# cristicbz/rust-doom

Measured on NVIDIA H100. Metric: frames/sec at 1920x1080 (palette-index bit-exact), higher is better.
Workload: dtype u8

## Files before the change

rust-doom_b200/csrc/b2d_kernels.cu:

```cuda
#include "b2d_kernels.cuh"

namespace b2d {

namespace {

constexpr unsigned kFull = 0xFFFFFFFFu;

constexpr int kMaskWords = 128;
constexpr int kStackDepth = 128;

constexpr uint32_t kVisBit = 1u << 25, kSolidBit = 1u << 24;
__device__ __forceinline__ uint32_t pack_range(int lo, int hi, uint32_t bits) {
    return (uint32_t)lo | ((uint32_t)hi << 12) | bits;
}
__device__ __forceinline__ int range_lo(uint32_t r) { return (int)(r & 0xFFFu); }
__device__ __forceinline__ int range_hi(uint32_t r) { return (int)((r >> 12) & 0xFFFu); }

__device__ __forceinline__ uint32_t word_bits(int w, int lo, int hi) {
    int a = max(lo, w * 32), b = min(hi, w * 32 + 31);
    if (a > b) return 0u;
    uint32_t m = 0xFFFFFFFFu >> (31 - (b - w * 32));
    return m & (0xFFFFFFFFu << (a - w * 32));
}

// ... 166 lines not shown
        if (--budget < 0) { status |= kStatusNoTermination; break; }
        uint32_t child = stack[--sp];
        __syncwarp();
        if (child & kLeaf) {
            uint32_t id = child & 0x7FFFFFFFu;
            if (id >= (uint32_t)sc.nss) continue;
            const int4 ssv = ssec_s[id];
            SSectorRec ss;
            ss.first_seg = ssv.x; ss.num_segs = ssv.y; ss.sector = ssv.z; ss.sprites = ssv.w;
            if (ss.sector < 0) continue;
            {
                const int sfirst = ss.sprites & 0xFFFFFF;
                int scnt = (ss.sprites >> 24) & 0xFF;
                if (sfirst + scnt > sc.nsprites) scnt = sc.nsprites > sfirst ? sc.nsprites - sfirst : 0;
                int nvis = 0;
                for (int k0 = 0; k0 < scnt; k0 += 32) {
                    const int k = k0 + lane, pi = sfirst + k;
                    const uint32_t r = k < scnt ? sprr[pi] : 0u;
                    const bool vis = (r & kVisBit) && lane_range_open(mask, range_lo(r), range_hi(r));
                    int rank = 0, total = 0;
                    const int32_t myz = vis ? sprz[pi] : 0;
                    for (int j0 = 0; j0 < scnt; j0 += 32) {
                        const int j = j0 + lane, pj = sfirst + j;
                        const uint32_t rj = j < scnt ? sprr[pj] : 0u;
                        const bool vj = (rj & kVisBit) && lane_range_open(mask, range_lo(rj), range_hi(rj));
                        const int32_t zj = vj ? sprz[pj] : 0;
                        unsigned mj = __ballot_sync(kFull, vj);
                        total += __popc(mj);
                        while (mj) {
                            const int b = __ffs(mj) - 1;
                            mj &= mj - 1;
                            const int32_t zb = __shfl_sync(kFull, zj, b);
                            const int jb = j0 + b;
                            if (vis && (zb < myz || (zb == myz && jb < k))) rank++;
                        }
                    }
                    const int pos = count + rank;
                    if (vis && pos < sc.nsegs + sc.nsprites) list[pos] = (uint16_t)(sc.nsegs + pi);
                    nvis = total;
                }
                count = min(count + nvis, sc.nsegs + sc.nsprites);
                __syncwarp();
            }
            for (int k0 = 0; k0 < ss.num_segs; k0 += 32) {
                int k = k0 + lane;
                int si = ss.first_seg + k;
                uint32_t r = k < ss.num_segs ? segr[si] : 0u;
                bool vis = (r & kVisBit) && lane_range_open(mask, range_lo(r), range_hi(r));
                unsigned m = __ballot_sync(kFull, vis);
                int pos = count + __popc(m & ((1u << lane) - 1u));
                if (vis && pos < sc.nsegs + sc.nsprites) list[pos] = (uint16_t)si;
                count = min(count + __popc(m), sc.nsegs + sc.nsprites);
                unsigned sm = __ballot_sync(kFull, vis && (r & kSolidBit));
                __syncwarp();
                while (sm) {
                    int j = __ffs(sm) - 1;
                    sm &= sm - 1;
                    uint32_t rj = __shfl_sync(kFull, r, j);
                    mark_solid(mask, lane, range_lo(rj), range_hi(rj), passes);
                }
                __syncwarp();
            }
            if (!range_open(mask, lane, 0, vw.W - 1, passes)) break;
        } else {
            if (child >= (uint32_t)sc.nnodes) continue;
            const int4 nl = node_s[2 * child], nc = node_s[2 * child + 1];
            int side = node_side(fc.pose, nl.x, nl.y, nl.z, nl.w);
            uint32_t near_c = (uint32_t)(side ? nc.y : nc.x), far_c = (uint32_t)(side ? nc.x : nc.y);
            uint32_t rn = boxr[2 * child + side], rf = boxr[2 * child + (side ^ 1)];
            bool far_vis = (rf & kVisBit) && range_open(mask, lane, range_lo(rf), range_hi(rf), passes);
            bool near_vis = (rn & kVisBit) && range_open(mask, lane, range_lo(rn), range_hi(rn), passes);
            int need = (far_vis ? 1 : 0) + (near_vis ? 1 : 0);
            if (sp + need > kStackDepth) { status = kStatusStackOverflow; break; }
            if (lane == 0) {
                int p = sp;
                if (far_vis) stack[p++] = far_c;
                if (near_vis) stack[p++] = near_c;
            }
            sp += need;
            __syncwarp();
        }
    }
    __syncwarp();
    if (warp == 0 && lane == 0) {
        if (count > stride) { count = stride; status |= kStatusWorklistFull; }
        s_count = count; s_status = status;
    }
    __syncthreads();
    count = s_count; status = s_status;

    for (int k = tid; k < count; k += nthr) {
        int si = list[k];
        SegFrame sf;
        if (si >= sc.nsegs) {
            const int pi = si - sc.nsegs;
            const SpriteRec &P = state_table<kStates>(sc.sprites, tb, st.off_sprites)[pi];
            SpriteFrame sp;
            sprite_setup(fc, vw, P.x, P.y, (int32_t)state_table<kStates>(sc.tex, tb, 0u)[P.tex].w, sp);
            sprite_entry(pi, sp, sf);
            work[(size_t)frame * stride + k] = sf;
            continue;
        }
        const SegRec &S = state_table<kStates>(sc.segs, tb, st.off_segs)[si];
        seg_frame_setup(vw, tx[S.v1], tz[S.v1], tx[S.v2], tz[S.v2], sf, false);
        sf.seg = si;
        work[(size_t)frame * stride + k] = sf;
    }
    if (tid == 0) {
        if (status) atomicOr(sc.status_flag, status);
        fc.count = count;
        fc.status = status;
#pragma unroll
        for (int i = 0; i < 6; i++) fc.pad[i] = 0;
        if (kStates) fc.pad[0] = (int32_t)slot;
        frames[frame] = fc;
    }
    __syncthreads();
    }
}

__device__ __forceinline__ uint32_t lds_u32(uint32_t a) {
    uint32_t v;
    asm("ld.shared.u32 %0, [%1];" : "=r"(v) : "r"(a));
    return v;
}

struct RasterCtx {
    const DeviceScene *sc;
    uint32_t pal_s;
    uint2 *rowz;
    PlaneDir dir;
    uint8_t *fb;
    uint32_t *rgba;
    int W, H, x, lane;
    uint32_t skycol;
};

template <bool kRgba>
__device__ __forceinline__ void put_px(const RasterCtx &c, uint8_t *p8, uint32_t *p32, bool on, uint32_t v) {
    if (on) {
        if (kRgba) {
            *p8 = (uint8_t)v;
            *p32 = lds_u32(c.pal_s + 4u * v);
        } else {
            __stcs(p8, (uint8_t)v);
        }
    }
}

__host__ __device__ __forceinline__ bool tex_interleaved(const TexRec &T) { return b2d::tex_interleaved(T.h, T.texel_off); }

constexpr int kBatch = 8;

template <bool kRgba, int kW>
__device__ __forceinline__ void store_batch(const RasterCtx &c, uint8_t *p8, uint32_t *p32, const uint32_t (&v)[kBatch],
                                            int y, int ya, int yb, bool full) {
    const int Wc = kW ? kW : c.W;
    if (full) {
#pragma unroll
        for (int k = 0; k < kBatch; k++) put_px<kRgba>(c, p8 + (size_t)k * Wc, kRgba ? p32 + (size_t)k * Wc : nullptr, true, v[k]);
    } else {
        const uint32_t m = row_mask(y, ya, yb, kBatch);
#pragma unroll
        for (int k = 0; k < kBatch; k++)
            put_px<kRgba>(c, p8 + (size_t)k * Wc, kRgba ? p32 + (size_t)k * Wc : nullptr, (m >> k) & 1u, v[k]);
    }
}

template <bool kRgba, int kW>
__device__ __forceinline__ void fill_void_warp(const RasterCtx &c, int ya, int yb) {
    bool act = ya < yb;
    int y0 = __reduce_min_sync(kFull, act ? ya : 0x7FFFFFFF);
    int y1 = __reduce_max_sync(kFull, act ? yb : 0);
    if (y0 >= y1) return;
    const int Wc = kW ? kW : c.W;
    uint8_t *p8 = c.fb + (size_t)y0 * Wc;
    uint32_t *p32 = kRgba ? c.rgba + (size_t)y0 * Wc : nullptr;
#pragma unroll 1
    for (int y = y0; y < y1; y++, p8 += Wc, p32 += Wc) put_px<kRgba>(c, p8, p32, y >= ya && y < yb, 0u);
}

template <bool kRgba, int kW>
__device__ __forceinline__ void draw_sky_warp(const RasterCtx &c, int ya, int yb) {
    const DeviceScene &sc = *c.sc;
    if (sc.sky_tex < 0) { fill_void_warp<kRgba, kW>(c, ya, yb); return; }
    const TexRec T = sc.tex[sc.sky_tex];
    const bool inter = tex_interleaved(T);
    const uint8_t *px = sc.lit_texels + T.texel_off + (inter ? 4u * c.skycol : c.skycol);
    const uint32_t w4 = 4u * T.w;
    bool act = ya < yb;
    int y0 = __reduce_min_sync(kFull, act ? ya : 0x7FFFFFFF);
    int y1 = __reduce_max_sync(kFull, act ? yb : 0);
    if (y0 >= y1) return;
    const int Wc = kW ? kW : c.W;
    uint8_t *p8 = c.fb + (size_t)y0 * Wc;
    uint32_t *p32 = kRgba ? c.rgba + (size_t)y0 * Wc : nullptr;
#pragma unroll 2
    for (int y = y0; y < y1; y++, p8 += Wc, p32 += Wc) {
        const uint32_t r = sc.skyrow[y];
        put_px<kRgba>(c, p8, p32, y >= ya && y < yb, __ldg(px + (inter ? (r >> 2) * w4 + (r & 3u) : r * T.w)));
    }
}

template <bool kRgba, int kW>
__device__ __forceinline__ void draw_plane_warp(const RasterCtx &c, const FrameConst &fc, const View &vw,
                                                int ya, int yb, int32_t h, int32_t flat, int lightb,
                                                bool visible) {
    const DeviceScene &sc = *c.sc;
    if (!__any_sync(kFull, ya < yb)) return;
    if (!visible) { fill_void_warp<kRgba, kW>(c, ya, yb); return; }
    if (flat == kFlatSky) { draw_sky_warp<kRgba, kW>(c, ya, yb); return; }
    if (flat < 0 || flat >= sc.nflats) { fill_void_warp<kRgba, kW>(c, ya, yb); return; }
    const uint64_t px_hi = reinterpret_cast<uint64_t>(sc.lit_flats) & 0xFFFFFFFF00000000ull;
    const uint32_t habs = plane_habs(h, fc.pose.z);
    bool act = ya < yb;
    int y0 = __reduce_min_sync(kFull, act ? ya : 0x7FFFFFFF);
    int y1 = __reduce_max_sync(kFull, act ? yb : 0);
    const int full_lo = __reduce_max_sync(kFull, act ? ya : 0x7FFFFFFF);
    const int full_hi = __reduce_min_sync(kFull, act ? yb : 0);
    const int Wc = kW ? kW : c.W;
    uint8_t *p8 = c.fb + (size_t)y0 * Wc;
    uint32_t *p32 = kRgba ? c.rgba + (size_t)y0 * Wc : nullptr;
    const uint32_t bu = (uint32_t)fc.pose.x << 10, bv = (uint32_t)fc.pose.y << 10;
    const uint32_t ax = (uint32_t)c.dir.ax, ay = (uint32_t)c.dir.ay;
    for (int yc = y0; yc < y1; yc += 32) {
        int yy = yc + c.lane;
        if (yy < y1) {
            const PlaneRow pr = plane_row(habs, sc.yslope[yy]);
            c.rowz[c.lane] = make_uint2(pr.z8q, (sc.lit_flat_stride >> 6) * (uint32_t)light_row(lightb, pr.z8) + 64u * (uint32_t)flat);
        }
        __syncwarp();
        const int rows = min(32, y1 - yc);
        int j = 0;
        for (; j + kBatch <= rows; j += kBatch, p8 += (size_t)kBatch * Wc, p32 += (size_t)kBatch * Wc) {
            uint32_t v[kBatch];
#pragma unroll
            for (int k = 0; k < kBatch; k++) {
                const uint2 rz = c.rowz[j + k];
                v[k] = __ldg(reinterpret_cast<const uint8_t *>(px_hi | flat_offset(rz.y, bu + rz.x * ax, bv + rz.x * ay)));
            }
            const int y = yc + j;
            store_batch<kRgba, kW>(c, p8, p32, v, y, ya, yb, y >= full_lo && y + kBatch <= full_hi);
        }
        for (; j < rows; j++, p8 += Wc, p32 += Wc) {
            const uint2 rz = c.rowz[j];
            const int y = yc + j;
            put_px<kRgba>(c, p8, p32, y >= ya && y < yb,
                          __ldg(reinterpret_cast<const uint8_t *>(px_hi | flat_offset(rz.y, bu + rz.x * ax, bv + rz.x * ay))));
        }
        __syncwarp();
    }
}

template <bool kRgba, int kW, int R>
__device__ __forceinline__ void wall_fast_loop(const RasterCtx &c, const uint8_t *plq, uint32_t w4, uint32_t nq, uint32_t q,
                                               uint32_t acc, uint32_t ts29, int y0, int y1, int ya, int yb,
                                               int full_lo, int full_hi) {
    const int Wc = kW ? kW : c.W;
    uint8_t *p8 = c.fb + (size_t)y0 * Wc;
    uint32_t *p32 = kRgba ? c.rgba + (size_t)y0 * Wc : nullptr;
    asm("" : "+l"(plq));
#pragma unroll 1
    for (int y = y0; y < y1; y += R, p8 += (size_t)R * Wc, p32 += (size_t)R * Wc) {
        const uint32_t q1 = q + 1u == nq ? 0u : q + 1u;
        const uint32_t w0 = __ldg(reinterpret_cast<const uint32_t *>(plq + (size_t)q * w4));
        const uint32_t w1 = __ldg(reinterpret_cast<const uint32_t *>(plq + (size_t)q1 * w4));
        if (y >= full_lo && y + R <= full_hi) {
#pragma unroll
            for (int k = 0; k < R; k++) {
                uint32_t v = pick_byte(w0, w1, wall_sel(acc, ts29, (uint32_t)k));
                if (kRgba) v &= 0xFFu;
                put_px<kRgba>(c, p8 + (size_t)k * Wc, kRgba ? p32 + (size_t)k * Wc : nullptr, true, v);
            }
        } else {
            const uint32_t m = row_mask(y, ya, yb, R);
#pragma unroll
            for (int k = 0; k < R; k++) {
                uint32_t v = pick_byte(w0, w1, wall_sel(acc, ts29, (uint32_t)k));
                if (kRgba) v &= 0xFFu;
                put_px<kRgba>(c, p8 + (size_t)k * Wc, kRgba ? p32 + (size_t)k * Wc : nullptr, (m >> k) & 1u, v);
            }
        }
        wall_advance(acc, q, ts29, (uint32_t)R, nq);
    }
}

template <bool kRgba, int kW>
__device__ __forceinline__ void draw_wall_warp(const RasterCtx &c, const FrameConst &fc, int ya, int yb,
                                               int32_t tex, int32_t tA, int32_t hA, int32_t ucol,
                                               int32_t iscale, int row) {
    const DeviceScene &sc = *c.sc;
    if (!__any_sync(kFull, ya < yb)) return;
    if (tex < 0 || tex >= sc.ntex) { fill_void_warp<kRgba, kW>(c, ya, yb); return; }
    const TexRec T = sc.tex[tex];
    bool act = ya < yb;
    const uint32_t col = (uint32_t)floormod32(ucol, (int32_t)T.w);
    const uint8_t *pl = sc.lit_texels + (size_t)row * sc.lit_texel_stride + T.texel_off;
    const uint32_t tstep = (uint32_t)(iscale >> 4);
    int y0 = __reduce_min_sync(kFull, act ? ya : 0x7FFFFFFF);
    int y1 = __reduce_max_sync(kFull, act ? yb : 0);
    const int full_lo = __reduce_max_sync(kFull, act ? ya : 0x7FFFFFFF);
    const int full_hi = __reduce_min_sync(kFull, act ? yb : 0);
    uint32_t t = (uint32_t)wall_tbase(tA, hA, fc.pose.z, c.H, iscale) + (uint32_t)y0 * tstep;
    const int Wc = kW ? kW : c.W;
    uint8_t *p8 = c.fb + (size_t)y0 * Wc;
    uint32_t *p32 = kRgba ? c.rgba + (size_t)y0 * Wc : nullptr;
    if (tex_interleaved(T) && T.h >= 8u) {
        const uint32_t ts = act ? tstep : 0u;
        const bool f16 = __all_sync(kFull, ts <= kWallFast16);
        if (f16 || __all_sync(kFull, ts <= kWallFast8)) {
            const uint32_t tt = act ? t : 0u;
            const uint32_t r0 = wall_row((int32_t)tt, T.h, T.hmagic, T.hbias);
            const uint8_t *plq = pl + 4u * col;
            if (f16) wall_fast_loop<kRgba, kW, 16>(c, plq, 4u * T.w, T.h >> 2, r0 >> 2, wall_acc29(tt, r0), ts << 13, y0, y1, ya, yb, full_lo, full_hi);
            else wall_fast_loop<kRgba, kW, 8>(c, plq, 4u * T.w, T.h >> 2, r0 >> 2, wall_acc29(tt, r0), ts << 13, y0, y1, ya, yb, full_lo, full_hi);
            return;
        }
    }
    if (tex_interleaved(T)) {
        const uint32_t colb = 4u * col, w4 = 4u * T.w;
        for (int y = y0; y < y1; y += kBatch, p8 += (size_t)kBatch * Wc, p32 += (size_t)kBatch * Wc, t += (uint32_t)kBatch * tstep) {
            const uint32_t r0 = wall_row((int32_t)t, T.h, T.hmagic, T.hbias);
            const uint32_t acc = wall_acc(t, r0);
            const uint32_t b7 = (acc + 7u * tstep) >> 16;
            uint32_t v[kBatch];
            if (__all_sync(kFull, b7 < 8u)) {
                const uint32_t q0 = r0 >> 2, q1 = next_quad(q0, T.h);
                const uint32_t w0 = __ldg(reinterpret_cast<const uint32_t *>(pl + (q0 * w4 + colb)));
                const uint32_t w1 = __ldg(reinterpret_cast<const uint32_t *>(pl + (q1 * w4 + colb)));
#pragma unroll
                for (int k = 0; k < kBatch; k++) {
                    v[k] = pick_byte(w0, w1, (acc + (uint32_t)k * tstep) >> 16);
                    if (kRgba) v[k] &= 0xFFu;
                }
            } else {
                const uint32_t t4 = t + 4u * tstep;
                const uint32_t r4 = wall_row((int32_t)t4, T.h, T.hmagic, T.hbias);
                const uint32_t acc4 = wall_acc(t4, r4);
                if (__all_sync(kFull, ((acc + 3u * tstep) >> 16) < 8u && ((acc4 + 3u * tstep) >> 16) < 8u)) {
                    const uint32_t q0 = r0 >> 2, q4 = r4 >> 2;
                    const uint32_t a0 = __ldg(reinterpret_cast<const uint32_t *>(pl + (q0 * w4 + colb)));
                    const uint32_t a1 = __ldg(reinterpret_cast<const uint32_t *>(pl + (next_quad(q0, T.h) * w4 + colb)));
                    const uint32_t b0 = __ldg(reinterpret_cast<const uint32_t *>(pl + (q4 * w4 + colb)));
                    const uint32_t b1 = __ldg(reinterpret_cast<const uint32_t *>(pl + (next_quad(q4, T.h) * w4 + colb)));
#pragma unroll
                    for (int k = 0; k < 4; k++) {
                        v[k] = pick_byte(a0, a1, (acc + (uint32_t)k * tstep) >> 16);
                        v[k + 4] = pick_byte(b0, b1, (acc4 + (uint32_t)k * tstep) >> 16);
                        if (kRgba) { v[k] &= 0xFFu; v[k + 4] &= 0xFFu; }
                    }
                } else {
#pragma unroll
                    for (int k = 0; k < kBatch; k++) {
                        const uint32_t rk = wall_row((int32_t)(t + (uint32_t)k * tstep), T.h, T.hmagic, T.hbias);
                        v[k] = __ldg(pl + ((rk >> 2) * w4 + colb + (rk & 3u)));
                    }
                }
            }
            store_batch<kRgba, kW>(c, p8, p32, v, y, ya, yb, y >= full_lo && y + kBatch <= full_hi);
        }
    } else {
        const uint8_t *px = pl + col;
#pragma unroll 1
        for (int y = y0; y < y1; y++, p8 += Wc, p32 += Wc, t += tstep)
            put_px<kRgba>(c, p8, p32, y >= ya && y < yb, __ldg(px + wall_row((int32_t)t, T.h, T.hmagic, T.hbias) * T.w));
    }
}

__device__ __forceinline__ uint32_t *masked_entry(const DeviceScene &sc, const uint32_t *chunks, int e) {
    return sc.masked_list + ((size_t)chunks[e / kMaskedChunk] * kMaskedChunk + (size_t)(e % kMaskedChunk)) * 33u;
}
__device__ __forceinline__ uint32_t *masked_push(const DeviceScene &sc, uint32_t *chunks, int &mcount, int lane) {
    bool ok = mcount < sc.masked_cap;
    if (ok && mcount % kMaskedChunk == 0) {
        uint32_t id = 0;
        if (lane == 0) id = atomicAdd(sc.masked_counter, 1u);
        id = __shfl_sync(kFull, id, 0);
        ok = id < sc.masked_chunks;
        if (ok && lane == 0) chunks[mcount / kMaskedChunk] = id;
        __syncwarp();
    }
    if (!ok) {
        if (lane == 0) atomicOr(sc.status_flag, kStatusMaskedFull);
        return nullptr;
    }
    return masked_entry(sc, chunks, mcount++);
}

template <bool kRgba, int kW, bool kStates>
__device__ __noinline__ void masked_pass(const DeviceScene &sc, const View &vw, int32_t pose_z, uint8_t *fb,
                                         uint32_t *rgba, uint32_t pal_s, int x, int lane,
                                         const SegFrame *wl, const uint32_t *chunks, int count) {
    RasterCtx c;
    c.sc = &sc; c.pal_s = pal_s; c.fb = fb; c.rgba = rgba;
    c.W = vw.W; c.H = vw.H; c.x = x; c.lane = lane;
    const int Wc = kW ? kW : c.W;
    for (int e = count - 1; e >= 0; e--) {
        const uint32_t *ml = masked_entry(sc, chunks, e);
        const uint32_t k = ml[0];
        const uint32_t packed = ml[1 + c.lane];
        int ya = (int)(packed & 0xFFFFu), yb = (int)(packed >> 16);
        const SegFrame sf = wl[k];
        int32_t tex, tA, hA, ucol = 0, iscale = 1, row = 0;
        if (is_sprite_entry(sf)) {
            SpriteFrame sp;
            const SpriteRec P = sc.sprites[entry_sprite(sf, sp)];
            if (P.tex < 0 || P.tex >= sc.ntex) continue;
            const int32_t sw = (int32_t)sc.tex[P.tex].w, sh = (int32_t)sc.tex[P.tex].h;
            const int64_t scale = sprite_scale(vw, sp.cz);
            int32_t z8;
            scale_depth(vw, scale, iscale, z8);
            row = light_row_sprite(P.light, z8);
            tex = P.tex; tA = 0; hA = P.low + sh;
            if (ya < yb) {
                clip_rows(P.low + sh, P.low, (int32_t)scale, pose_z, c.H, ya, yb);
                ucol = sprite_column(sp, vw, c.x, sw);
            }
        } else {
            const SegRec S = sc.segs[sf.seg];
            if (S.mid < 0 || S.mid >= sc.nmids) continue;
            const MidRec M = sc.mids[S.mid];
            tex = M.tex; tA = M.t_high; hA = M.high;
            ColumnEval ce = {0u, 1, 1, 0};
            if (ya < yb && column_eval(sf, vw, c.x, ce)) {
                clip_rows(M.high, M.low, ce.scale, pose_z, c.H, ya, yb);
                ucol = wall_column(S.uoff, S.len_q12, ce.s24);
                iscale = ce.iscale;
                row = light_row(S.light, ce.z8);
            } else {
                ya = yb = 0;
            }
        }
        if (tex < 0 || tex >= sc.ntex) continue;
        const TexRec T = sc.tex[tex];
        const bool act = ya < yb;
        int y0 = __reduce_min_sync(kFull, act ? ya : 0x7FFFFFFF);
        int y1 = __reduce_max_sync(kFull, act ? yb : 0);
        if (y0 >= y1) continue;
        const uint32_t col = (uint32_t)floormod32(ucol, (int32_t)T.w);
        const bool inter = tex_interleaved(T);
        const bool has_mask = T.mask_off != 0xFFFFFFFFu;
        const uint8_t *pl = sc.lit_texels + (size_t)row * sc.lit_texel_stride + T.texel_off;
        const uint8_t *pm = sc.lit_texels + (size_t)32 * sc.lit_texel_stride + T.texel_off;
        const uint32_t tstep = (uint32_t)(iscale >> 4);
        uint32_t t = (uint32_t)wall_tbase(tA, hA, pose_z, c.H, iscale) + (uint32_t)y0 * tstep;
        uint8_t *p8 = c.fb + (size_t)y0 * Wc;
        uint32_t *p32 = kRgba ? c.rgba + (size_t)y0 * Wc : nullptr;
        const uint32_t len = act ? (uint32_t)(yb - ya) : 0u;
        if (inter) {
            const uint32_t colb = 4u * col, w4 = 4u * T.w;
#pragma unroll 1
            for (int y = y0; y < y1; y += kBatch, p8 += (size_t)kBatch * Wc, p32 += (size_t)kBatch * Wc, t += (uint32_t)kBatch * tstep) {
                const uint32_t r0 = wall_row((int32_t)t, T.h, T.hmagic, T.hbias);
                const uint32_t acc = wall_acc(t, r0);
                const uint32_t d = (uint32_t)(y - ya);
                uint32_t v[kBatch], o[kBatch];
                if (__all_sync(kFull, ((acc + 7u * tstep) >> 16) < 8u)) {
                    const uint32_t o0 = (r0 >> 2) * w4 + colb, o1 = next_quad(r0 >> 2, T.h) * w4 + colb;
                    const uint32_t w0 = __ldg(reinterpret_cast<const uint32_t *>(pl + o0));
                    const uint32_t w1 = __ldg(reinterpret_cast<const uint32_t *>(pl + o1));
                    uint32_t m0 = 0x01010101u, m1 = 0x01010101u;
                    if (has_mask) {
                        m0 = __ldg(reinterpret_cast<const uint32_t *>(pm + o0));
                        m1 = __ldg(reinterpret_cast<const uint32_t *>(pm + o1));
                    }
#pragma unroll
                    for (int k = 0; k < kBatch; k++) {
                        const uint32_t bk = (acc + (uint32_t)k * tstep) >> 16;
                        v[k] = pick_byte(w0, w1, bk) & 0xFFu;
                        o[k] = pick_byte(m0, m1, bk) & 0xFFu;
                    }
                } else {
#pragma unroll
                    for (int k = 0; k < kBatch; k++) {
                        const uint32_t rk = wall_row((int32_t)(t + (uint32_t)k * tstep), T.h, T.hmagic, T.hbias);
                        const uint32_t off = (rk >> 2) * w4 + colb + (rk & 3u);
                        v[k] = __ldg(pl + off);
                        o[k] = has_mask ? (uint32_t)__ldg(pm + off) : 1u;
                    }
                }
#pragma unroll
                for (int k = 0; k < kBatch; k++)
                    put_px<kRgba>(c, p8 + (size_t)k * Wc, kRgba ? p32 + (size_t)k * Wc : nullptr, d + (uint32_t)k < len && o[k] != 0u, v[k]);
            }
        } else {
#pragma unroll 1
            for (int y = y0; y < y1; y++, p8 += Wc, p32 += Wc, t += tstep) {
                const uint32_t off = wall_row((int32_t)t, T.h, T.hmagic, T.hbias) * T.w + col;
                const bool on = (uint32_t)(y - ya) < len && (!has_mask || __ldg(pm + off) != 0);
                put_px<kRgba>(c, p8, p32, on, __ldg(pl + off));
            }
        }
    }
}

constexpr int kRasterWarps = 4;

template <bool kRgba, int kW, bool kMasked, bool kStates>
__global__ void __launch_bounds__(32 * kRasterWarps, 16 / kRasterWarps)
b2d_raster_kernel(const __grid_constant__ DeviceScene sc, const __grid_constant__ View vw, const FrameConst *__restrict__ frames,
                  const SegFrame *__restrict__ work, int stride, int n, int strips,
                  uint8_t *__restrict__ index_fb, uint32_t *__restrict__ rgba_fb, const __grid_constant__ StateTables st) {
    __shared__ uint32_t s_pal[kRgba ? 256 : 1];
    __shared__ uint2 s_rowz[kRasterWarps][32];
    __shared__ uint32_t s_chunks[kRasterWarps][kMasked ? kMaskedCapMax / kMaskedChunk : 1];
    if (kRgba) {
        for (int i = threadIdx.x; i < 256; i += blockDim.x) s_pal[i] = sc.palette[i];
        __syncthreads();
    }

    const int lane = threadIdx.x & 31;
    const long long gw = (long long)blockIdx.x * (blockDim.x >> 5) + (threadIdx.x >> 5);
    if (gw >= (long long)n * strips) return;
    const int frame = (int)(gw / strips), strip = (int)(gw % strips);
    const int W = kW ? kW : vw.W, H = vw.H;
    const int x0 = strip * 32, x = x0 + lane;
    const bool inside = x < W;

    const FrameConst fc = frames[frame];
    const DeviceScene *scp = &sc;
    if constexpr (kStates) {
        __shared__ DeviceScene s_sc[kRasterWarps];
        DeviceScene *d = &s_sc[threadIdx.x >> 5];
        const uint32_t *src = reinterpret_cast<const uint32_t *>(&sc);
        uint32_t *dst = reinterpret_cast<uint32_t *>(d);
        for (int i = lane; i < (int)(sizeof(DeviceScene) / 4); i += 32) dst[i] = src[i];
        __syncwarp();
        if (lane == 0) {
            const uint8_t *tb = st.base + (size_t)(uint32_t)fc.pad[0] * st.slot_bytes;
            d->tex = reinterpret_cast<const TexRec *>(tb);
            d->sectors = reinterpret_cast<const SectorRec *>(tb + st.off_sectors);
            d->segs = reinterpret_cast<const SegRec *>(tb + st.off_segs);
            d->sprites = reinterpret_cast<const SpriteRec *>(tb + st.off_sprites);
            d->mids = reinterpret_cast<const MidRec *>(tb + st.off_mids);
        }
        __syncwarp();
        scp = d;
    }
    const DeviceScene &ts = *scp;
    RasterCtx c;
    c.sc = &ts;
    c.pal_s = (uint32_t)__cvta_generic_to_shared(s_pal);
    c.rowz = s_rowz[threadIdx.x >> 5];
    c.dir = plane_dir(fc, vw, inside ? x : 0, sc.invF);
    c.fb = index_fb + (size_t)frame * W * H + (inside ? x : 0);
    c.rgba = kRgba ? rgba_fb + (size_t)frame * W * H + (inside ? x : 0) : nullptr;
    c.W = W; c.H = H; c.x = x; c.lane = lane;
    c.skycol = 0;
    if (sc.sky_tex >= 0 && inside) c.skycol = umulhi32(sky_u32(x, vw, fc.pose.angle), ts.tex[sc.sky_tex].w);

    int ct = 0, cb = inside ? H : 0;
    uint32_t *chunks = s_chunks[threadIdx.x >> 5];
    asm("" : "+l"(chunks));
    const bool defer = kMasked && sc.masked_list != nullptr;
    int mcount = 0;
    const SegFrame *wl = work + (size_t)frame * stride;
    const int count = fc.count;
    bool done = false;

    for (int k0 = 0; k0 < count && !done; k0 += 32) {
        int k = k0 + lane;
        bool overlap = false;
        if (k < count) {
            int xlo = wl[k].xlo, xhi = wl[k].xhi;
            overlap = xhi >= x0 && xlo <= x0 + 31;
        }
        unsigned m = __ballot_sync(kFull, overlap);
        while (m) {
            int j = __ffs(m) - 1;
            m &= m - 1;
            if (!__any_sync(kFull, ct < cb)) { done = true; break; }
            const SegFrame sf = wl[k0 + j];
            bool in = inside && ct < cb && x >= sf.xlo && x <= sf.xhi;
            if (!__any_sync(kFull, in)) continue;
            if (is_sprite_entry(sf)) {
                if (defer) {
                    uint32_t *ml = masked_push(sc, chunks, mcount, lane);
                    if (ml) {
                        if (lane == 0) ml[0] = (uint32_t)(k0 + j);
                        ml[1 + lane] = in ? ((uint32_t)ct | ((uint32_t)cb << 16)) : 0u;
                    }
                }
                continue;
            }
            ColumnEval ce = {0u, 1, 1, 0};
            bool ok = in && column_eval(sf, vw, x, ce);
            if (!__any_sync(kFull, ok)) continue;

            const SegRec S = ts.segs[sf.seg];
            const SectorRec SF = ts.sectors[S.front];
            const int32_t fcl = SF.ceil, ffl = SF.floor;
            const bool two = S.flags & kSegTwoSided;
            const bool ceil_vis = plane_visible(true, fcl, SF.ceil_flat == kFlatSky, fc.pose.z);
            const bool floor_vis = plane_visible(false, ffl, SF.floor_flat == kFlatSky, fc.pose.z);

            WallRows wr = {ct, ct, ct, ct};
            int yend = ct, row = 0;
            int32_t ucol = 0;
            if (ok) {
                row = light_row(S.light, ce.z8);
                ucol = wall_column(S.uoff, S.len_q12, ce.s24);
                wr = wall_rows(fcl, ffl, two, S.otop, S.obot, ce.scale, fc.pose.z, H, ct, cb);
                yend = cb;
            }
#pragma unroll 1
            for (int pz = 0; pz < 2; pz++) {
                const bool top = pz == 0;
                draw_plane_warp<kRgba, kW>(c, fc, vw, ok ? (top ? ct : wr.y4) : 0, ok ? (top ? wr.y1 : yend) : 0,
                                                    top ? fcl : ffl, top ? SF.ceil_flat : SF.floor_flat, SF.light,
                                                    top ? ceil_vis : floor_vis);
            }
#pragma unroll 1
            for (int pw = 0; pw < 2; pw++) {
                const bool upper = pw == 0;
                if (!wall_piece(upper, two, fcl, ffl, S.otop, S.obot)) continue;
                draw_wall_warp<kRgba, kW>(c, fc, ok ? (upper ? wr.y1 : wr.y3) : 0, ok ? (upper ? wr.y2 : wr.y4) : 0,
                                                   upper ? S.texA : S.texB, upper ? S.tA : S.tB, upper ? S.hA : S.hB,
                                                   ucol, ce.iscale, row);
            }
            if (ok) wall_window(two, wr, H, ct, cb);
            if (defer && two && S.mid >= 0) {
                const bool keep = ok && wr.y2 < wr.y3;
                if (__any_sync(kFull, keep)) {
                    uint32_t *ml = masked_push(sc, chunks, mcount, lane);
                    if (ml) {
                        if (lane == 0) ml[0] = (uint32_t)(k0 + j);
                        ml[1 + lane] = keep ? ((uint32_t)wr.y2 | ((uint32_t)wr.y3 << 16)) : 0u;
                    }
                }
            }
        }
    }
    fill_void_warp<kRgba, kW>(c, inside ? ct : 0, inside ? cb : 0);
    if (kMasked && mcount > 0) {
        __syncwarp();
        masked_pass<kRgba, kW, kStates>(ts, vw, fc.pose.z, c.fb, c.rgba, c.pal_s, x, lane, wl, chunks, mcount);
    }
}

__global__ void __launch_bounds__(256)
b2d_palette_kernel(const uint32_t *__restrict__ palette, const uint8_t *__restrict__ index,
                   uint32_t *__restrict__ rgba, size_t n_pixels) {
    __shared__ uint32_t s_pal[256];
    s_pal[threadIdx.x] = palette[threadIdx.x];
    __syncthreads();
    const bool aligned = ((reinterpret_cast<uintptr_t>(index) | reinterpret_cast<uintptr_t>(rgba)) & 15) == 0;
    const size_t nvec = aligned ? n_pixels / 16 : 0;
    const size_t stride = (size_t)gridDim.x * blockDim.x;
    for (size_t i = (size_t)blockIdx.x * blockDim.x + threadIdx.x; i < nvec; i += stride) {
        uint4 in = __ldcs(reinterpret_cast<const uint4 *>(index) + i);
        uint32_t wds[4] = {in.x, in.y, in.z, in.w};
        uint4 *out = reinterpret_cast<uint4 *>(rgba) + 4 * i;
#pragma unroll
        for (int q = 0; q < 4; q++) {
            uint4 o;
            o.x = s_pal[wds[q] & 0xFF];
            o.y = s_pal[(wds[q] >> 8) & 0xFF];
            o.z = s_pal[(wds[q] >> 16) & 0xFF];
            o.w = s_pal[wds[q] >> 24];
            __stcs(out + q, o);
        }
    }
    for (size_t p = nvec * 16 + (size_t)blockIdx.x * blockDim.x + threadIdx.x; p < n_pixels; p += stride)
        rgba[p] = s_pal[index[p]];
}

}

size_t walk_smem_per_warp(const DeviceScene &sc) { return walk_layout(sc.nverts, sc.nsegs, sc.nnodes, sc.nss, sc.nsprites).total; }

static int device_sms() {
    int dev = 0, sms = 0;
    cudaGetDevice(&dev);
    cudaDeviceGetAttribute(&sms, cudaDevAttrMultiProcessorCount, dev);
    return sms > 0 ? sms : 1;
}

cudaError_t launch_walk(const DeviceScene &sc, const View &vw, const Pose *d_poses, int n,
                        FrameConst *d_frames, SegFrame *d_work, int stride, cudaStream_t stream, bool background,
                        const StateTables *states) {
    if (n <= 0) return cudaSuccess;
    const size_t smem = walk_smem_per_warp(sc);
    if (smem > 227 * 1024) return cudaErrorInvalidValue;
    if (smem > 48 * 1024) {
        cudaError_t e = states ? cudaFuncSetAttribute(b2d_walk_kernel<true>, cudaFuncAttributeMaxDynamicSharedMemorySize, (int)smem)
                               : cudaFuncSetAttribute(b2d_walk_kernel<false>, cudaFuncAttributeMaxDynamicSharedMemorySize, (int)smem);
        if (e != cudaSuccess) return e;
    }
    const int sms = device_sms();
    const int blocks = (background && n > sms) ? sms : n, warps = 4;
    const StateTables none{};
    if (states) b2d_walk_kernel<true><<<blocks, warps * 32, smem, stream>>>(sc, vw, d_poses, n, d_frames, d_work, stride, *states);
    else b2d_walk_kernel<false><<<blocks, warps * 32, smem, stream>>>(sc, vw, d_poses, n, d_frames, d_work, stride, none);
    return cudaGetLastError();
}

cudaError_t launch_raster(const DeviceScene &sc, const View &vw, const FrameConst *d_frames,
                          const SegFrame *d_work, int stride, int n, uint8_t *d_index_fb,
                          uint32_t *d_rgba, cudaStream_t stream, const StateTables *states) {
    if (n <= 0) return cudaSuccess;
    const int strips = (vw.W + 31) / 32;
    const int nblocks = (int)(((long long)n * strips + kRasterWarps - 1) / kRasterWarps);
    const bool masked = (sc.nmids > 0 || sc.nsprites > 0) && sc.masked_list;
    const StateTables none{};
#define B2D_RASTER_GO2(RGBA, KW, KS) do { \
    if (masked) b2d_raster_kernel<RGBA, KW, true, KS><<<nblocks, 32 * kRasterWarps, 0, stream>>>(sc, vw, d_frames, d_work, stride, n, strips, d_index_fb, d_rgba, KS ? *states : none); \
    else b2d_raster_kernel<RGBA, KW, false, KS><<<nblocks, 32 * kRasterWarps, 0, stream>>>(sc, vw, d_frames, d_work, stride, n, strips, d_index_fb, d_rgba, KS ? *states : none); \
    } while (0)
#define B2D_RASTER_GO(RGBA, KW) do { if (states) B2D_RASTER_GO2(RGBA, KW, true); else B2D_RASTER_GO2(RGBA, KW, false); } while (0)
    if (d_rgba) { if (vw.W == 1920) B2D_RASTER_GO(true, 1920); else B2D_RASTER_GO(true, 0); }
    else if (vw.W == 1920) B2D_RASTER_GO(false, 1920);
    else if (vw.W == 3840) B2D_RASTER_GO(false, 3840);
    else B2D_RASTER_GO(false, 0);
#undef B2D_RASTER_GO
#undef B2D_RASTER_GO2
    return cudaGetLastError();
}

namespace {
__global__ void __launch_bounds__(256)
b2d_prelight_kernel(const uint8_t *__restrict__ colormap, const uint8_t *__restrict__ src, uint8_t *__restrict__ dst,
                    size_t n, size_t stride) {
    __shared__ uint8_t cm[32 * 256];
    for (int i = threadIdx.x; i < 32 * 256; i += blockDim.x) cm[i] = colormap[i];
    __syncthreads();
    for (size_t i = (size_t)blockIdx.x * blockDim.x + threadIdx.x; i < n; i += (size_t)gridDim.x * blockDim.x) {
        const uint32_t t = src[i];
#pragma unroll 4
        for (int r = 0; r < 32; r++) dst[(size_t)r * stride + i] = cm[r * 256 + t];
    }
}
}

namespace {
__global__ void __launch_bounds__(256)
b2d_prelight_tex_kernel(const uint8_t *__restrict__ colormap, const uint8_t *__restrict__ texels,
                        const TexRec *__restrict__ tex, int ntex, uint8_t *__restrict__ dst, size_t stride) {
    __shared__ uint8_t cm[32 * 256];
    for (int i = threadIdx.x; i < 32 * 256; i += blockDim.x) cm[i] = colormap[i];
    __syncthreads();
    for (int ti = blockIdx.x; ti < ntex; ti += gridDim.x) {
        const TexRec T = tex[ti];
        const bool inter = tex_interleaved(T);
        const uint32_t n = T.w * T.h;
        for (uint32_t i = threadIdx.x; i < n; i += blockDim.x) {
            const uint32_t row = i / T.w, col = i - row * T.w;
            const uint32_t o = lit_index(inter, T.w, row, col);
            const uint32_t t = texels[T.texel_off + i];
            for (int r = 0; r < 32; r++) dst[(size_t)r * stride + T.texel_off + o] = cm[r * 256 + t];
            if (T.mask_off != 0xFFFFFFFFu) dst[(size_t)32 * stride + T.texel_off + o] = texels[T.mask_off + i];
        }
    }
}
}

cudaError_t launch_prelight_textures(const uint8_t *d_colormap, const uint8_t *d_texels, const TexRec *d_tex, int ntex,
                                     uint8_t *d_dst, size_t stride, cudaStream_t stream) {
    if (ntex <= 0) return cudaSuccess;
    const int cap = device_sms() * 8;
    b2d_prelight_tex_kernel<<<ntex < cap ? ntex : cap, 256, 0, stream>>>(d_colormap, d_texels, d_tex, ntex, d_dst, stride);
    return cudaGetLastError();
// ... 59 lines not shown
```

rust-doom_b200/csrc/b2d_math.cuh:

```cuda
#pragma once
#include <stdint.h>

#if defined(__CUDACC__)
#define B2D_HD __host__ __device__ __forceinline__
#else
#define B2D_HD inline
#endif

namespace b2d {

struct Pose { int32_t x, y, z; uint32_t angle; };
struct View { int32_t W, H, F, FY2; };

struct FrameConst {
    Pose pose;
    int32_t cosq, sinq;
    int32_t px8, py8;
    int32_t count;
    int32_t status;
    int32_t pad[6];
};
static_assert(sizeof(FrameConst) == 64, "FrameConst");

constexpr int32_t kStatusStackOverflow = 1;
// ... 166 lines not shown
    sf.sh = (int16_t)sh;
    sf.e = (int16_t)(5 - sh + shm);
    sf.Dmax = M >> 8;
    sf.flags = 0;
    if (want_noskip) {
        ColumnEval ce;
        bool ok = column_eval(sf, vw, (int)lo, ce) && column_eval(sf, vw, (int)hi, ce);
        sf.flags = ok ? kSegFrameNoSkip : 0;
    }
    sf.pad = 0;
    return true;
}

B2D_HD bool seg_closes(bool two, int32_t otop, int32_t obot) { return !two || otop <= obot; }
B2D_HD bool seg_solid(bool closes, const SegFrame &sf) { return closes && (sf.flags & kSegFrameNoSkip); }

B2D_HD int light_row(int b, int32_t z8) {
    uint32_t Z = (uint32_t)z8 + 720u;
    int32_t num = (int32_t)(64u * (uint32_t)(255 - b) * Z) - 5875200;
    if (num <= 0) return 0;
    uint32_t r = (uint32_t)num / (255u * Z);
    return r > 31u ? 31 : (int)r;
}

B2D_HD int yrow(int32_t h, int32_t scale, int32_t pose_z, int32_t H) {
    int64_t hrel8 = ((int64_t)h << 8) - (int64_t)(pose_z >> 8);
    int64_t Y = ((int64_t)H << 25) - hrel8 * scale;
    int64_t r = (Y + ((int64_t)1 << 25) - 1) >> 26;
    return (int)clampv<int64_t>(r, 0, H);
}

B2D_HD bool plane_visible(bool ceiling, int32_t h, bool sky, int32_t pose_z) {
    const int64_t h16 = (int64_t)h << 16;
    return (ceiling ? h16 > pose_z : h16 < pose_z) || sky;
}
struct WallRows { int y1, y2, y3, y4; };
B2D_HD WallRows wall_rows(int32_t ceil, int32_t floor, bool two, int32_t otop, int32_t obot, int32_t scale, int32_t pose_z,
                          int32_t H, int ct, int cb) {
    WallRows r;
    const int yfc = yrow(ceil, scale, pose_z, H), yff = yrow(floor, scale, pose_z, H);
    r.y1 = clampv(yfc, ct, cb);
    if (!two) {
        r.y2 = clampv(yff, r.y1, cb);
        r.y3 = r.y2; r.y4 = r.y2;
    } else {
        r.y2 = clampv(yrow(otop, scale, pose_z, H), r.y1, cb);
        r.y3 = clampv(yrow(obot, scale, pose_z, H), r.y2, cb);
        r.y4 = clampv(yff, r.y3, cb);
    }
    return r;
}
B2D_HD bool wall_piece(bool upper, bool two, int32_t ceil, int32_t floor, int32_t otop, int32_t obot) {
    return upper ? (!two || otop < ceil) : (two && obot > floor);
}
B2D_HD void wall_window(bool two, const WallRows &r, int32_t H, int &ct, int &cb) {
    if (!two || r.y2 >= r.y3) { ct = H; cb = 0; }
    else { ct = r.y2; cb = r.y3; }
}
B2D_HD int32_t wall_column(int32_t uoff, int32_t len_q12, uint32_t s24) {
    return uoff + (int32_t)(((uint64_t)s24 * (uint32_t)len_q12) >> 36);
}
B2D_HD void clip_rows(int32_t high, int32_t low, int32_t scale, int32_t pose_z, int32_t H, int &ya, int &yb) {
    const int a = yrow(high, scale, pose_z, H), b = yrow(low, scale, pose_z, H);
    if (a > ya) ya = a;
    if (b < yb) yb = b;
}

B2D_HD uint32_t yslope_entry(int y, const View &vw) {
    int32_t r2 = 2 * y + 1 - vw.H;
    if (r2 < 0) r2 = -r2;
    if (r2 == 0) r2 = 1;
    return (uint32_t)(((uint64_t)vw.FY2 << 16) / (uint32_t)r2);
}

B2D_HD uint32_t plane_habs(int32_t h, int32_t pose_z) {
    int64_t hrel = clampv<int64_t>(((int64_t)h << 16) - pose_z, -((int64_t)1 << 27), (int64_t)1 << 27);
    return (uint32_t)(hrel < 0 ? -hrel : hrel);
}
B2D_HD int32_t wall_hrel(int32_t h, int32_t pose_z) {
    return (int32_t)clampv<int64_t>(((int64_t)h << 16) - pose_z, -((int64_t)1 << 27), (int64_t)1 << 27);
}

struct PlaneDir { int32_t ax, ay; };
B2D_HD PlaneDir plane_dir(const FrameConst &f, const View &vw, int x, uint32_t invF) {
    const int64_t c2 = 2 * (int64_t)x + 1 - vw.W;
    const int64_t nx = ((int64_t)f.cosq * vw.F + (int64_t)f.sinq * c2) >> 4;
    const int64_t ny = ((int64_t)f.sinq * vw.F - (int64_t)f.cosq * c2) >> 4;
    PlaneDir d;
    d.ax = (int32_t)((nx * (int64_t)invF) >> 40);
    d.ay = (int32_t)((ny * (int64_t)invF) >> 40);
    return d;
}
struct PlaneRow { uint32_t z8q; int32_t z8; };
B2D_HD PlaneRow plane_row(uint32_t habs, uint32_t yslope) {
    PlaneRow pr;
    uint64_t zz = ((uint64_t)habs * yslope) >> 16;
    int32_t z16 = zz > 0x7FFFFFFFull ? 0x7FFFFFFF : (int32_t)zz;
    pr.z8q = (uint32_t)(z16 >> 8);
    int32_t z8 = z16 >> 13;
    pr.z8 = z8 > 65535 ? 65535 : z8;
    return pr;
}
B2D_HD uint32_t plane_u(int32_t pose_xy, uint32_t z8q, int32_t a) { return ((uint32_t)pose_xy << 10) + z8q * (uint32_t)a; }
B2D_HD uint32_t flat_index(uint32_t U, uint32_t V) { return ((U >> 26) << 6) | (V >> 26); }
B2D_HD uint32_t flat_offset(uint32_t cm6, uint32_t U, uint32_t V) {
#if defined(__CUDA_ARCH__)
    return __funnelshift_l(V, cm6 + (U >> 26), 6);
#else
    return ((cm6 + (U >> 26)) << 6) | (V >> 26);
#endif
}

B2D_HD int32_t wall_tbase(int32_t tA, int32_t hA, int32_t pose_z, int32_t H, int32_t iscale) {
    int64_t t = ((int64_t)tA << 16) + wall_hrel(hA, pose_z) + (((int64_t)(1 - H) * iscale) >> 5);
    return (int32_t)t;
}
B2D_HD uint32_t wall_row(int32_t t, uint32_t h, uint32_t hmagic, uint32_t hbias) {
    uint32_t n = ((uint32_t)t + (hbias << 16)) >> 16;
    uint32_t q = umulhi32(n, hmagic);
    return n - q * h;
}

B2D_HD bool tex_interleaved(uint32_t h, uint32_t texel_off) { return (h & 3u) == 0u && (texel_off & 3u) == 0u && h <= 4096u; }
B2D_HD uint32_t lit_index(bool inter, uint32_t w, uint32_t row, uint32_t col) {
    return inter ? ((row >> 2) * w + col) * 4u + (row & 3u) : row * w + col;
}
B2D_HD uint32_t wall_acc(uint32_t t, uint32_t r0) { return (t & 0xFFFFu) | ((r0 & 3u) << 16); }
B2D_HD uint32_t next_quad(uint32_t q0, uint32_t h) { return q0 + 1u == (h >> 2) ? 0u : q0 + 1u; }
B2D_HD uint32_t pick_byte(uint32_t lo, uint32_t hi, uint32_t sel) {
#if defined(__CUDA_ARCH__)
    uint32_t d;
    asm("prmt.b32 %0, %1, %2, %3;" : "=r"(d) : "r"(lo), "r"(hi), "r"(sel));
    return d;
#else
    return ((sel & 4u) ? hi : lo) >> (8u * (sel & 3u)) & 0xFFu;
#endif
}

constexpr uint32_t kWallFast8 = 32768u;
constexpr uint32_t kWallFast16 = 16384u;
B2D_HD uint32_t wall_acc29(uint32_t t, uint32_t r0) { return ((r0 & 3u) << 29) | ((t & 0xFFFFu) << 13); }
B2D_HD uint32_t wall_sel(uint32_t acc, uint32_t ts29, uint32_t k) { return (acc + k * ts29) >> 29; }
B2D_HD void wall_advance(uint32_t &acc, uint32_t &q, uint32_t ts29, uint32_t R, uint32_t nq) {
    acc += R * ts29;
    q += acc >> 31;
    if (q >= nq) q -= nq;
    acc &= 0x7FFFFFFFu;
}
B2D_HD uint32_t row_mask(int y, int ya, int yb, int R) {
    int lo = ya - y, hi = yb - y;
    if (lo < 0) lo = 0;
    if (hi > R) hi = R;
    if (hi <= lo) return 0u;
    return ((1u << hi) - 1u) & ~((1u << lo) - 1u);
}

B2D_HD uint32_t sky_u32(int x, const View &vw, uint32_t angle) {
    uint64_t num = ((uint64_t)(2 * x + 1)) << 32;
    return (uint32_t)(num / (uint32_t)vw.W) - (angle << 3);
}
B2D_HD int32_t sky_row(int y, int32_t H, int32_t skyh) {
    int32_t r = 2 * y + 1;
    if (r < H) return (r * skyh) / H;
    return floormod32(((2 * H - r) * skyh) / H, skyh);
}

constexpr int32_t kBoxNearQ8 = 32 * 256;
B2D_HD bool box_range(const FrameConst &f, const View &vw, const int32_t box[4], int &lo, int &hi) {
    bool all_behind = true, any_near = false;
    int64_t mn = 0x7FFFFFFFFFFFFFFFLL, mx = -0x7FFFFFFFFFFFFFFFLL;
    for (int i = 0; i < 4; i++) {
        int32_t tx, tz;
        to_view(f, box[2 + (i & 1)], box[i >> 1], tx, tz);
        if (tz >= -256) all_behind = false;
        if (tz < kBoxNearQ8) { any_near = true; continue; }
        int64_t c = floordiv64((int64_t)tx * vw.F, tz);
        int64_t xc = floordiv64(c - 1 + vw.W, 2);
        if (xc < mn) mn = xc;
        if (xc > mx) mx = xc;
    }
    if (all_behind) return false;
    if (any_near) { lo = 0; hi = vw.W - 1; return true; }
    mn -= 2; mx += 2;
    if (mx < 0 || mn > vw.W - 1) return false;
    lo = (int)(mn < 0 ? 0 : mn);
    hi = (int)(mx > vw.W - 1 ? vw.W - 1 : mx);
    return true;
}

B2D_HD int light_row_sprite(int b, int32_t z8) {
    int32_t r1 = (32 * (255 - b)) / 255;
    uint32_t Z = (uint32_t)z8 + 800u;
    int32_t num = (int32_t)(64u * (uint32_t)(255 - b) * Z) - 6528000;
    int32_t r2 = num <= 0 ? 0 : (int32_t)((uint32_t)num / (255u * Z));
    int32_t r = r1 > r2 ? r1 : r2;
    return r > 31 ? 31 : r;
}

struct SpriteFrame {
    int64_t cx, cz;
    int32_t lo, hi;
    int32_t scale, iscale, z8;
};

B2D_HD int64_t sprite_scale(const View &vw, int64_t cz) {
    const int64_t scale = ((int64_t)vw.FY2 << 25) / cz, cap = (int64_t)vw.FY2 << 17;
    return scale > cap ? cap : scale;
}

B2D_HD bool sprite_setup(const FrameConst &f, const View &vw, int32_t x, int32_t y, int32_t w, SpriteFrame &sp) {
    int32_t tx, tz;
    to_view(f, x, y, tx, tz);
    sp.cx = tx; sp.cz = tz;
    if (tz < 256) return false;
    const int64_t F = vw.F, W = vw.W;
    const int64_t L = (sp.cx - (int64_t)w * 128) * F, R = (sp.cx + (int64_t)w * 128) * F;
    int64_t lo = 0, hi = W - 1;
    constrain(lo, hi, sp.cz * (1 - W) - L, 2 * sp.cz, 0);
    constrain(lo, hi, R - 1 - sp.cz * (1 - W), -2 * sp.cz, 0);
    if (lo > hi) return false;
    sp.lo = (int32_t)lo; sp.hi = (int32_t)hi;
    const int64_t scale = sprite_scale(vw, sp.cz);
    if (scale < 1) return false;
    sp.scale = (int32_t)scale;
    scale_depth(vw, scale, sp.iscale, sp.z8);
    return true;
}

B2D_HD void sprite_entry(int sprite, const SpriteFrame &sp, SegFrame &sf) {
    sf.Nc = sp.cx; sf.Nx = sp.cz; sf.Dc = 0; sf.Dx = 0; sf.Dmax = 0; sf.Rm = 0; sf.sh = 0; sf.e = 0;
    sf.seg = -1 - sprite; sf.xlo = (int16_t)sp.lo; sf.xhi = (int16_t)sp.hi; sf.flags = 0; sf.pad = 0;
}
B2D_HD bool is_sprite_entry(const SegFrame &sf) { return sf.seg < 0; }
B2D_HD int entry_sprite(const SegFrame &sf, SpriteFrame &sp) {
    sp.cx = sf.Nc; sp.cz = sf.Nx;
    return -1 - sf.seg;
}

constexpr int kMaskedCapMax = 128;
B2D_HD int strip_masked_cap(int nmids, int nsprites) { return clampv(nmids + nsprites, 8, kMaskedCapMax); }

B2D_HD int32_t sprite_column(const SpriteFrame &sp, const View &vw, int x, int32_t w) {
    const int64_t c2 = 2 * (int64_t)x + 1 - vw.W;
    const int64_t L = (sp.cx - (int64_t)w * 128) * vw.F;
    return (int32_t)clampv<int64_t>(floordiv64(sp.cz * c2 - L, 256 * (int64_t)vw.F), 0, w - 1);
}

}
```

Before: 507,900.

## Batch void/sky stores, double-buffer plane row setup, prefetch wall quads

Void fill and sky drawing now go through the batched store path, eight rows at a time, with full-warp fast masks. Plane drawing double-buffers the per-row shared-memory setup, computing the next 32 rows while the current ones are still being fetched. It also uses a larger row batch for non-RGBA paths (16 or 32 rows). The wall fast loop prefetches the next texel quads before storing the current ones, and row_mask is fixed to handle a 32-row width. Together these aim to raise memory-level parallelism and hide load latency, at the cost of doubled shared rowz storage and more registers.

```diff
diff --git a/rust-doom_b200/csrc/b2d_kernels.cu b/rust-doom_b200/csrc/b2d_kernels.cu
--- a/rust-doom_b200/csrc/b2d_kernels.cu
+++ b/rust-doom_b200/csrc/b2d_kernels.cu
@@ -342,17 +342,17 @@
 
 constexpr int kBatch = 8;
 
-template <bool kRgba, int kW>
-__device__ __forceinline__ void store_batch(const RasterCtx &c, uint8_t *p8, uint32_t *p32, const uint32_t (&v)[kBatch],
+template <bool kRgba, int kW, int R = kBatch>
+__device__ __forceinline__ void store_batch(const RasterCtx &c, uint8_t *p8, uint32_t *p32, const uint32_t (&v)[R],
                                             int y, int ya, int yb, bool full) {
     const int Wc = kW ? kW : c.W;
     if (full) {
 #pragma unroll
-        for (int k = 0; k < kBatch; k++) put_px<kRgba>(c, p8 + (size_t)k * Wc, kRgba ? p32 + (size_t)k * Wc : nullptr, true, v[k]);
+        for (int k = 0; k < R; k++) put_px<kRgba>(c, p8 + (size_t)k * Wc, kRgba ? p32 + (size_t)k * Wc : nullptr, true, v[k]);
     } else {
-        const uint32_t m = row_mask(y, ya, yb, kBatch);
-#pragma unroll
-        for (int k = 0; k < kBatch; k++)
+        const uint32_t m = row_mask(y, ya, yb, R);
+#pragma unroll
+        for (int k = 0; k < R; k++)
             put_px<kRgba>(c, p8 + (size_t)k * Wc, kRgba ? p32 + (size_t)k * Wc : nullptr, (m >> k) & 1u, v[k]);
     }
 }
@@ -363,11 +363,15 @@
     int y0 = __reduce_min_sync(kFull, act ? ya : 0x7FFFFFFF);
     int y1 = __reduce_max_sync(kFull, act ? yb : 0);
     if (y0 >= y1) return;
+    const int full_lo = __reduce_max_sync(kFull, act ? ya : 0x7FFFFFFF);
+    const int full_hi = __reduce_min_sync(kFull, act ? yb : 0);
     const int Wc = kW ? kW : c.W;
     uint8_t *p8 = c.fb + (size_t)y0 * Wc;
     uint32_t *p32 = kRgba ? c.rgba + (size_t)y0 * Wc : nullptr;
+    const uint32_t v[kBatch] = {};
 #pragma unroll 1
-    for (int y = y0; y < y1; y++, p8 += Wc, p32 += Wc) put_px<kRgba>(c, p8, p32, y >= ya && y < yb, 0u);
+    for (int y = y0; y < y1; y += kBatch, p8 += (size_t)kBatch * Wc, p32 += (size_t)kBatch * Wc)
+        store_batch<kRgba, kW>(c, p8, p32, v, y, ya, yb, y >= full_lo && y + kBatch <= full_hi);
 }
 
 template <bool kRgba, int kW>
@@ -382,17 +386,24 @@
     int y0 = __reduce_min_sync(kFull, act ? ya : 0x7FFFFFFF);
     int y1 = __reduce_max_sync(kFull, act ? yb : 0);
     if (y0 >= y1) return;
+    const int full_lo = __reduce_max_sync(kFull, act ? ya : 0x7FFFFFFF);
+    const int full_hi = __reduce_min_sync(kFull, act ? yb : 0);
     const int Wc = kW ? kW : c.W;
     uint8_t *p8 = c.fb + (size_t)y0 * Wc;
     uint32_t *p32 = kRgba ? c.rgba + (size_t)y0 * Wc : nullptr;
-#pragma unroll 2
-    for (int y = y0; y < y1; y++, p8 += Wc, p32 += Wc) {
-        const uint32_t r = sc.skyrow[y];
-        put_px<kRgba>(c, p8, p32, y >= ya && y < yb, __ldg(px + (inter ? (r >> 2) * w4 + (r & 3u) : r * T.w)));
-    }
-}
-
-template <bool kRgba, int kW>
+#pragma unroll 1
+    for (int y = y0; y < y1; y += kBatch, p8 += (size_t)kBatch * Wc, p32 += (size_t)kBatch * Wc) {
+        uint32_t v[kBatch];
+#pragma unroll
+        for (int k = 0; k < kBatch; k++) {
+            const uint32_t r = sc.skyrow[min(y + k, y1 - 1)];
+            v[k] = __ldg(px + (inter ? (r >> 2) * w4 + (r & 3u) : r * T.w));
+        }
+        store_batch<kRgba, kW>(c, p8, p32, v, y, ya, yb, y >= full_lo && y + kBatch <= full_hi);
+    }
+}
+
+template <bool kRgba, int kW, int R>
 __device__ __forceinline__ void draw_plane_warp(const RasterCtx &c, const FrameConst &fc, const View &vw,
                                                 int ya, int yb, int32_t h, int32_t flat, int lightb,
                                                 bool visible) {
@@ -413,32 +424,46 @@
     uint32_t *p32 = kRgba ? c.rgba + (size_t)y0 * Wc : nullptr;
     const uint32_t bu = (uint32_t)fc.pose.x << 10, bv = (uint32_t)fc.pose.y << 10;
     const uint32_t ax = (uint32_t)c.dir.ax, ay = (uint32_t)c.dir.ay;
-    for (int yc = y0; yc < y1; yc += 32) {
-        int yy = yc + c.lane;
+    const uint32_t cm_row = sc.lit_flat_stride >> 6, cm_flat = 64u * (uint32_t)flat;
+    auto prepare = [&](int yc, uint2 *rowz) {
+        const int yy = yc + c.lane;
         if (yy < y1) {
             const PlaneRow pr = plane_row(habs, sc.yslope[yy]);
-            c.rowz[c.lane] = make_uint2(pr.z8q, (sc.lit_flat_stride >> 6) * (uint32_t)light_row(lightb, pr.z8) + 64u * (uint32_t)flat);
-        }
-        __syncwarp();
+            rowz[c.lane] = make_uint2(pr.z8q, cm_row * (uint32_t)light_row(lightb, pr.z8) + cm_flat);
+        }
+    };
+    auto texel = [&](const uint2 &rz) -> uint32_t {
+        return __ldg(reinterpret_cast<const uint8_t *>(px_hi | flat_offset(rz.y, bu + rz.x * ax, bv + rz.x * ay)));
+    };
+    uint2 *rz_cur = c.rowz, *rz_next = c.rowz + 32;
+    prepare(y0, rz_cur);
+    __syncwarp();
+    for (int yc = y0; yc < y1; yc += 32) {
         const int rows = min(32, y1 - yc);
         int j = 0;
-        for (; j + kBatch <= rows; j += kBatch, p8 += (size_t)kBatch * Wc, p32 += (size_t)kBatch * Wc) {
-            uint32_t v[kBatch];
-#pragma unroll
-            for (int k = 0; k < kBatch; k++) {
-                const uint2 rz = c.rowz[j + k];
-                v[k] = __ldg(reinterpret_cast<const uint8_t *>(px_hi | flat_offset(rz.y, bu + rz.x * ax, bv + rz.x * ay)));
-            }
+        for (; j + R <= rows; j += R, p8 += (size_t)R * Wc, p32 += (size_t)R * Wc) {
+            uint32_t v[R];
+#pragma unroll
+            for (int k = 0; k < R; k++) v[k] = texel(rz_cur[j + k]);
+            if (j == 0 && yc + 32 < y1) prepare(yc + 32, rz_next);
             const int y = yc + j;
-            store_batch<kRgba, kW>(c, p8, p32, v, y, ya, yb, y >= full_lo && y + kBatch <= full_hi);
+            store_batch<kRgba, kW, R>(c, p8, p32, v, y, ya, yb, y >= full_lo && y + R <= full_hi);
+        }
+        if (R > kBatch) {
+            for (; j + kBatch <= rows; j += kBatch, p8 += (size_t)kBatch * Wc, p32 += (size_t)kBatch * Wc) {
+                uint32_t v[kBatch];
+#pragma unroll
+                for (int k = 0; k < kBatch; k++) v[k] = texel(rz_cur[j + k]);
+                const int y = yc + j;
+                store_batch<kRgba, kW>(c, p8, p32, v, y, ya, yb, y >= full_lo && y + kBatch <= full_hi);
+            }
         }
         for (; j < rows; j++, p8 += Wc, p32 += Wc) {
-            const uint2 rz = c.rowz[j];
             const int y = yc + j;
-            put_px<kRgba>(c, p8, p32, y >= ya && y < yb,
-                          __ldg(reinterpret_cast<const uint8_t *>(px_hi | flat_offset(rz.y, bu + rz.x * ax, bv + rz.x * ay))));
+            put_px<kRgba>(c, p8, p32, y >= ya && y < yb, texel(rz_cur[j]));
         }
         __syncwarp();
+        uint2 *t = rz_cur; rz_cur = rz_next; rz_next = t;
     }
 }
 
@@ -450,15 +475,23 @@
     uint8_t *p8 = c.fb + (size_t)y0 * Wc;
     uint32_t *p32 = kRgba ? c.rgba + (size_t)y0 * Wc : nullptr;
     asm("" : "+l"(plq));
+    auto load_quads = [&](uint32_t qq, uint32_t &lo, uint32_t &hi) {
+        const uint32_t qq1 = qq + 1u == nq ? 0u : qq + 1u;
+        lo = __ldg(reinterpret_cast<const uint32_t *>(plq + (size_t)qq * w4));
+        hi = __ldg(reinterpret_cast<const uint32_t *>(plq + (size_t)qq1 * w4));
+    };
+    uint32_t w0, w1;
+    load_quads(q, w0, w1);
 #pragma unroll 1
     for (int y = y0; y < y1; y += R, p8 += (size_t)R * Wc, p32 += (size_t)R * Wc) {
-        const uint32_t q1 = q + 1u == nq ? 0u : q + 1u;
-        const uint32_t w0 = __ldg(reinterpret_cast<const uint32_t *>(plq + (size_t)q * w4));
-        const uint32_t w1 = __ldg(reinterpret_cast<const uint32_t *>(plq + (size_t)q1 * w4));
+        const uint32_t acc_b = acc;
+        wall_advance(acc, q, ts29, (uint32_t)R, nq);
+        uint32_t n0, n1;
+        if (!kRgba) load_quads(q, n0, n1);
         if (y >= full_lo && y + R <= full_hi) {
 #pragma unroll
             for (int k = 0; k < R; k++) {
-                uint32_t v = pick_byte(w0, w1, wall_sel(acc, ts29, (uint32_t)k));
+                uint32_t v = pick_byte(w0, w1, wall_sel(acc_b, ts29, (uint32_t)k));
                 if (kRgba) v &= 0xFFu;
                 put_px<kRgba>(c, p8 + (size_t)k * Wc, kRgba ? p32 + (size_t)k * Wc : nullptr, true, v);
             }
@@ -466,12 +499,13 @@
             const uint32_t m = row_mask(y, ya, yb, R);
 #pragma unroll
             for (int k = 0; k < R; k++) {
-                uint32_t v = pick_byte(w0, w1, wall_sel(acc, ts29, (uint32_t)k));
+                uint32_t v = pick_byte(w0, w1, wall_sel(acc_b, ts29, (uint32_t)k));
                 if (kRgba) v &= 0xFFu;
                 put_px<kRgba>(c, p8 + (size_t)k * Wc, kRgba ? p32 + (size_t)k * Wc : nullptr, (m >> k) & 1u, v);
             }
         }
-        wall_advance(acc, q, ts29, (uint32_t)R, nq);
+        if (kRgba) load_quads(q, n0, n1);
+        w0 = n0; w1 = n1;
     }
 }
 
@@ -692,7 +726,7 @@
                   const SegFrame *__restrict__ work, int stride, int n, int strips,
                   uint8_t *__restrict__ index_fb, uint32_t *__restrict__ rgba_fb, const __grid_constant__ StateTables st) {
     __shared__ uint32_t s_pal[kRgba ? 256 : 1];
-    __shared__ uint2 s_rowz[kRasterWarps][32];
+    __shared__ uint2 s_rowz[kRasterWarps][64];
     __shared__ uint32_t s_chunks[kRasterWarps][kMasked ? kMaskedCapMax / kMaskedChunk : 1];
     if (kRgba) {
         for (int i = threadIdx.x; i < 256; i += blockDim.x) s_pal[i] = sc.palette[i];
@@ -743,6 +777,7 @@
     uint32_t *chunks = s_chunks[threadIdx.x >> 5];
     asm("" : "+l"(chunks));
     const bool defer = kMasked && sc.masked_list != nullptr;
+    constexpr int kPlaneRows = kRgba ? kBatch : kMasked ? 16 : 32;
     int mcount = 0;
     const SegFrame *wl = work + (size_t)frame * stride;
     const int count = fc.count;
@@ -796,7 +831,7 @@
 #pragma unroll 1
             for (int pz = 0; pz < 2; pz++) {
                 const bool top = pz == 0;
-                draw_plane_warp<kRgba, kW>(c, fc, vw, ok ? (top ? ct : wr.y4) : 0, ok ? (top ? wr.y1 : yend) : 0,
+                draw_plane_warp<kRgba, kW, kPlaneRows>(c, fc, vw, ok ? (top ? ct : wr.y4) : 0, ok ? (top ? wr.y1 : yend) : 0,
                                                     top ? fcl : ffl, top ? SF.ceil_flat : SF.floor_flat, SF.light,
                                                     top ? ceil_vis : floor_vis);
             }
diff --git a/rust-doom_b200/csrc/b2d_math.cuh b/rust-doom_b200/csrc/b2d_math.cuh
--- a/rust-doom_b200/csrc/b2d_math.cuh
+++ b/rust-doom_b200/csrc/b2d_math.cuh
@@ -342,7 +342,7 @@
     if (lo < 0) lo = 0;
     if (hi > R) hi = R;
     if (hi <= lo) return 0u;
-    return ((1u << hi) - 1u) & ~((1u << lo) - 1u);
+    return (hi == 32 ? 0xFFFFFFFFu : (1u << hi) - 1u) & ~((1u << lo) - 1u);
 }
 
 B2D_HD uint32_t sky_u32(int x, const View &vw, uint32_t angle) {
```

Result: faster. 536,000, median of 6 (+5.5%).
